# megapose6d/megapose6d

Hardware: AMD Instinct MI355X
Metric: pose-hypotheses/sec (render+coarse+refine), 640×480, megapose-1.0-RGB (higher is better)
Workload: dtype f32 (results of fp32 arithmetic; the convolutions' multiplications run on the bf16 MFMA as EXACT piece products of the fp32 operands, fp32 accumulate)

## Files before the change

### include/mp_engine_debug.h

```cpp
#ifndef MP_ENGINE_DEBUG_H
#define MP_ENGINE_DEBUG_H

#include "mp_engine.h"

#ifdef __cplusplus
extern "C" {
#endif

int mp_clock_probe(double ms_target, double* shader_mhz, double* mfma_tflops, mp_stream stream);

int mp_conv_clock_read(double* shader_mhz, int reset);

int mp_conv_wino_stats(double* direct_flops, double* executed_flops, int reset);

int mp_conv_wino_bf16_stats(double* direct_flops, double* executed_bf16_flops, int reset);
int mp_conv_wino_bf16_clock(double* shader_mhz, double* cycles_per_step, int reset);
int mp_conv_wino_bf16_phases(double* prologue_cycles, double* epilogue_cycles);
int mp_conv_wino_bf16_telemetry(int on);

int mp_conv_stem_bg_stats(double* background_wgs, double* total_wgs, int reset);

#ifdef __cplusplus
}
#endif

#endif
```

### megapose6d_amd/_lib.py

```python
from __future__ import annotations

import ctypes as C
import os
from pathlib import Path

_HERE = Path(__file__).resolve().parent
LIB_PATH = _HERE / "libmp_engine.so"


class EngineError(RuntimeError):
    pass


class MeshDesc(C.Structure):
    _fields_ = [
        ("h_vertices", C.c_void_p),
        ("h_normals", C.c_void_p),
        ("h_colors", C.c_void_p),
        ("h_faces", C.c_void_p),
        ("n_vertices", C.c_int32),
        ("n_faces", C.c_int32),
    ]


# ... 61 lines not shown
    "mp_profile_query_ex": (_i, [_i, C.c_char_p, _i, C.POINTER(_i64), C.POINTER(C.c_double), C.POINTER(C.c_double), C.POINTER(C.c_double),
                                 C.POINTER(C.c_double), C.POINTER(C.c_double)]),
    "mp_device_info": (_i, [C.POINTER(_i), C.POINTER(_i), C.c_char_p, _i]),
    "mp_mesh_db_create": (_i, [C.POINTER(MeshDesc), _i, C.POINTER(_vp)]),
    "mp_mesh_db_set_texture": (_i, [_vp, _i, _vp, _vp, _i, _i, _i]),
    "mp_mesh_db_destroy": (_i, [_vp]),
    "mp_mesh_db_max_vertices": (_i, [_vp]),
    "mp_mesh_db_radius": (_f, [_vp, _i]),
    "mp_raster_workspace_bytes": (_sz, [_vp, _i, _i, _i]),
    "mp_raster_render": (_i, [_vp, _vp, _vp, _vp, _i, _i, _i, _u32, C.POINTER(Lights), _vp, _i64, _i, _i64, _i64, _i64, _i, _i, _i,
                              _vp, _sz, _vp]),
    "mp_raster_render_crop": (_i, [_vp, _vp, _vp, _vp, _i, _i, _i, _u32, C.POINTER(Lights), _vp, _i64, _i, _i64, _i64, _i64, _i, _i, _i,
                                   _vp, _sz, _vp, _i, _i, _i, _i, _i, _vp, _vp, _i, _vp]),
    "mp_raster_render_xrec": (_i, [_vp, _vp, _vp, _vp, _i, _i, _i, _u32, C.POINTER(Lights), _vp, _i64, _i, _i64, _i64, _i64, _i, _i, _i,
                                   _vp, _sz, _vp, _i, _i, _i, _i, _i, _vp, _vp, _u32, _vp, _i, _vp]),
    "mp_raster_job_flags": (_vp, [_vp, _vp, _i, _i, _i]),
    "mp_pack_observation_nhwc4": (_i, [_vp, _i, _i, _i, _i, _vp, _vp]),
    "mp_raster_scene_workspace_bytes": (_sz, [_vp, _i, _i, _i]),
    "mp_raster_render_scene": (_i, [_vp, _i, C.POINTER(C.c_int32), _vp, _vp, _vp, _vp, _vp, _vp, _i, _i, _u32, _vp, _i64, _i64, _i64, _i, _i,
                                    _i, _vp, _vp, _sz, _vp]),
    "mp_crop_roi_align": (_i, [_vp, _i, _i, _i, _i, _vp, _vp, _i, _i, _i, _vp, _i64, _i64, _i64, _i, _vp]),
    "mp_normalize_depth": (_i, [_vp, _i, _i, _i, _i, _i, C.POINTER(C.c_int32), _i, _vp, _i, _vp]),
    "mp_normalize_depth_f16": (_i, [_vp, _i, _i, _i, _i, _i, C.POINTER(C.c_int32), _i, _vp, _i, _vp]),
    "mp_conv_packed_floats": (_sz, [_i, _i, _i, _i]),
    "mp_conv_pack_weights": (_i, [_vp, _i, _i, _i, _i, _i, _vp, _vp]),
    "mp_conv2d_nhwc": (_i, [C.POINTER(ConvDesc), _vp]),
    "mp_conv2d_plan": (_i, [C.POINTER(ConvDesc), _i, C.POINTER(C.c_int32)]),
    "mp_conv_bf16x9_packed_bytes": (_sz, [_i, _i, _i, _i]),
    "mp_conv_bf16x9_pack_weights": (_i, [_vp, _i, _i, _i, _i, _i, _vp, _vp]),
    "mp_conv2d_bf16x9_nhwc": (_i, [C.POINTER(ConvDesc), _vp, _vp]),
    "mp_conv2d_kernel_name": (C.c_char_p, [C.POINTER(ConvDesc)]),
    "mp_conv_wino_packed_floats": (_sz, [_i, _i]),
    "mp_conv_wino_pack_weights": (_i, [_vp, _i, _i, _i, _vp, _vp]),
    "mp_conv_wino_eligible": (_i, [C.POINTER(ConvDesc), _i]),
    "mp_conv3x3_wino_nhwc": (_i, [C.POINTER(ConvDesc), _vp, _vp]),
    "mp_conv_wino_stats": (_i, [C.POINTER(C.c_double), C.POINTER(C.c_double), _i]),
    "mp_conv_wino_bf16_packed_bytes": (_sz, [_i, _i]),
    "mp_conv_wino_bf16_pack_weights": (_i, [_vp, _i, _i, _i, _vp, _vp]),
    "mp_conv3x3_wino_bf16_nhwc": (_i, [C.POINTER(ConvDesc), _vp, _vp]),
    "mp_conv_wino_bf16_stats": (_i, [C.POINTER(C.c_double), C.POINTER(C.c_double), _i]),
    "mp_conv_wino_bf16_clock": (_i, [C.POINTER(C.c_double), C.POINTER(C.c_double), _i]),
    "mp_conv_wino_bf16_phases": (_i, [C.POINTER(C.c_double), C.POINTER(C.c_double)]),
    "mp_conv_wino_bf16_telemetry": (_i, [_i]),
    "mp_xrec_elements": (_i, [_i, _i]),
    "mp_conv_stem_supported": (_i, [_i, _i, _i]),
    "mp_conv_stem_packed_bytes": (_sz, [_i, _i, _i, _i]),
    "mp_conv_stem_pack_weights": (_i, [_vp, _i, _i, _i, _i, _vp, _vp]),
    "mp_conv_stem_pack_weights_mask": (_i, [_vp, _i, _i, _i, _u32, _vp, _vp]),
    "mp_conv_stem_sparse_chunks": (_i, [_i, _i, _i]),
    "mp_conv_stem_sparse_packed_bytes": (_sz, [_i, _i, _i, _i]),
    "mp_conv_stem_pack_weights_sparse": (_i, [_vp, _i, _i, _i, _i, _vp, _vp]),
    "mp_conv_stem_xrec_sparse": (_i, [C.POINTER(ConvDesc), _vp, _vp, _i, _vp, _vp, _i, _vp]),
    "mp_conv_stem_bg_stats": (_i, [C.POINTER(C.c_double), C.POINTER(C.c_double), _i]),
    "mp_conv_stem_xrec": (_i, [C.POINTER(ConvDesc), _vp, _i, _vp]),
    "mp_conv_stem_xrec_pool": (_i, [C.POINTER(ConvDesc), _vp, _i, _vp, _i, _vp]),
    "mp_maxpool3x3s2": (_i, [_vp, _i, _i, _i, _i, _i, _vp, _i, _vp, _vp, _vp, _vp]),
    "mp_bn_relu_nhwc": (_i, [_vp, _i, _i, _i, _i, _i, _vp, _vp, _vp, _vp]),
    "mp_pool_fc_heads": (_i, [_vp, _i, _i, _i, _i, _i, _vp, _vp, _i, _vp, _vp, _i, _vp, _vp, _vp, _vp]),
    "mp_backbone_create": (_i, [_i, _i, _i, _i, C.POINTER(NamedTensor), _i, C.POINTER(_vp)]),
    "mp_backbone_create_wide": (_i, [_i, _i, _i, _i, _i, C.POINTER(NamedTensor), _i, C.POINTER(_vp)]),
    "mp_backbone_destroy": (_i, [_vp]),
    "mp_backbone_input_channels_padded": (_i, [_vp]),
    "mp_backbone_input_border": (_i, [_vp]),
    "mp_backbone_workspace_bytes": (_sz, [_vp, _i, _i, _i]),
    "mp_backbone_workspace_reset": (_i, [_vp, _vp]),
    "mp_backbone_forward": (_i, [_vp, _vp, _i, _i, _i, _vp, _vp, _vp, _vp, _sz, _vp]),
    "mp_backbone_forward_f16": (_i, [_vp, _vp, _i, _i, _i, _vp, _vp, _vp, _vp, _sz, _vp]),
    "mp_backbone_xrec_elements": (_i, [_vp, _i]),
    "mp_backbone_forward_xrec": (_i, [_vp, _vp, _i, _i, _i, _i, _vp, _vp, _vp, _vp, _sz, _vp]),
    "mp_backbone_xrec_prepare": (_i, [_vp, _u32]),
    "mp_backbone_forward_xrec_mask": (_i, [_vp, _vp, _u32, _i, _i, _i, _vp, _vp, _vp, _vp, _sz, _vp]),
    "mp_backbone_forward_xrec_sparse": (_i, [_vp, _vp, _u32, _vp, _i, _i, _i, _vp, _vp, _vp, _vp, _sz, _vp]),
    "mp_backbone_flops": (C.c_double, [_vp, _i, _i, _i]),
    "mp_normalize_T": (_i, [_vp, _i, _vp, _vp]),
    "mp_init_extents": (_i, [_vp, _i, _i, _vp, _i, _vp, _vp]),
    "mp_init_poses_from_boxes": (_i, [_vp, _vp, _vp, _vp, _vp, _i, _vp, _i, _vp, _vp]),
    "mp_pose_prepare": (_i, [_vp, _vp, _vp, _vp, _i, _i, _i, _i, _i, _i, _i, _i, _i, _i, _f, _vp, _vp, _vp, _vp, _vp, _vp,
                             _vp]),
    "mp_pose_multiview_n_views": (_i, [_i]),
    "mp_pose_prepare_ex": (_i, [_vp, _vp, _vp, _vp, _i, _i, _i, _i, _i, _i, _i, _i, _i, _i, _f, _vp, _vp, _vp, _vp, _vp, _vp, _vp, _vp]),
    "mp_pose_error_workspace_bytes": (_sz, [_i, _i, _i]),
    "mp_pose_error_sym": (_i, [_vp, _vp, _vp, _vp, _i, _vp, _i, _vp, _vp, _i, _i, _i, _i, _vp, _vp, _vp, _vp, _vp, _vp, _vp, _sz, _vp]),
    "mp_pose_error_nn": (_i, [_vp, _vp, _vp, _i, _vp, _vp, _i, _i, _i, _vp, _vp, _vp, _vp, _vp, _sz, _vp]),
    "mp_pose_error_rigid": (_i, [_vp, _vp, _i, _vp, _vp, _i, _vp, _vp, _i, _vp, _vp, _vp, _vp]),
    "mp_pose_error_mspd": (_i, [_vp, _vp, _vp, _vp, _i, _vp, _i, _vp, _vp, _i, _i, _i, _i, _vp, _vp, _vp, _vp, _vp, _vp, _vp, _sz, _vp]),
    "mp_vsd_workspace_bytes": (_sz, [_i, _i]),
    "mp_vsd": (_i, [_vp, _vp, _vp, _vp, _vp, _vp, _i, _i, _i, _vp, _vp, _i, _i, _i, _f, _vp, _i, _i, _i, _vp, _vp, _vp, _sz, _vp]),
    "mp_gt_info_workspace_bytes": (_sz, [_i]),
    "mp_gt_info": (_i, [_vp, _vp, _vp, _vp, _i, _i, _vp, _i, _i, _i, _i, _f, _i, _vp, _vp, _vp, _vp, _vp, _vp, _sz, _vp]),
    "mp_bop_match_limits": (_i, [C.POINTER(_i), C.POINTER(_i), C.POINTER(_i), C.POINTER(_i)]),
    "mp_bop_match_workspace_bytes": (_sz, [_i, _i, _i]),
    "mp_bop_match": (_i, [_vp, _vp, _vp, _vp, _vp, _vp, _vp, _vp, _vp, _vp, _i, _i, _i, _i, _i, _i, _i, _vp, _vp, _sz, _vp]),
    "mp_icp_workspace_bytes": (_sz, [_i, _i, _i, _i]),
    "mp_icp_refine": (_i, [_vp, _i, _vp, _vp, _vp, _vp, _vp, _i, _i, _i, _i, _i, _f, _i, _i, _vp, _vp, _vp, _vp, _sz, _vp]),
    "mp_icp_nn_max_points": (_i, []),
    "mp_icp_nn_workspace_bytes": (_sz, [_i, _i, _i, _i]),
    "mp_icp_refine_nn": (_i, [_vp, _i, _vp, _vp, _vp, _vp, _vp, _i, _i, _i, _i, _i, _f, _i, _vp, _vp, _vp, _vp, _vp, _vp, _sz, _vp]),
    "mp_pose_update": (_i, [_vp, _vp, _i, _vp, _vp, _i, _vp, _vp]),
    "mp_detector_default_config": (_i, [C.POINTER(DetectorConfig), _i, _i, _i]),
    "mp_detector_state_spec": (_i, [_i, _i, C.c_char_p, _i, C.POINTER(_i64), C.POINTER(C.c_int32)]),
    "mp_detector_create": (_i, [C.POINTER(DetectorConfig), C.POINTER(NamedTensor), _i, C.POINTER(_vp)]),
    "mp_detector_destroy": (_i, [_vp]),
    "mp_detector_workspace_bytes": (_sz, [_vp, _i, _i, _i]),
    "mp_detector_forward": (_i, [_vp, _vp, _i, _i, _i, _vp, _vp, _vp, _vp, _vp, _vp, _sz, _vp]),
    "mp_detector_debug_tensor": (_i, [_vp, C.c_char_p, C.POINTER(_vp), C.POINTER(_i64), C.POINTER(C.c_int32), C.POINTER(_i64), C.POINTER(_i64)]),
}
# ... 34 lines not shown
```

### megapose6d_amd/csrc/conv_stem.hip

```cpp
#include <cstdlib>
#include <vector>

#include "bf16x9_split.h"
#include "common.h"

namespace mp {
namespace stem {

typedef float f32x4 __attribute__((ext_vector_type(4)));
typedef __bf16 bf16x8 __attribute__((ext_vector_type(8)));
typedef unsigned u32x4 __attribute__((ext_vector_type(4)));

constexpr int TH = 8, TW = 16;
constexpr int NCO = 64;

struct Params {
  const unsigned char* __restrict__ x;
  const unsigned char* __restrict__ w;
  const float* __restrict__ bias;
  float* __restrict__ y;
  int N, Ho, Wo;
  int Hp, Wp;
  int in_off;
  int Cout, Hop, Wop, out_border;
  int tiles_x, tiles_y, n_cb;
  int n_steps;
  int relu;
  unsigned img_bytes;
  unsigned out_bytes;
  float* __restrict__ ypool;
  int Hq, Wq, pool_border;
  const unsigned char* __restrict__ tile_flags;
  const unsigned char* __restrict__ w_sparse;
  int fl_tx, fl_ty, q_use, n_steps_sparse;
  int H, W, pad;
  int count_bg;
};

__device__ unsigned long long g_stem_bg[2];

constexpr size_t LDS_PER_WG = 80 * 1024;

template <int KS, int Q>
struct Geo {
  static constexpr int PH = 2 * (TH - 1) + KS, PW = 2 * (TW - 1) + KS;
  static constexpr int QP = (Q % 2 == 0 && (size_t)(PH + 1) * ((PW * (Q + 1)) | 1) * 16 <= LDS_PER_WG) ? Q + 1 : Q;
  static constexpr int ROW16 = PW * QP;
  static constexpr int PITCH16 = ROW16 | 1;
  static constexpr int PITCH = PITCH16 * 16;
  static constexpr int KWQ = KS * Q;
  static constexpr int S = KS * KWQ;
  static constexpr int T = ((S + 3) / 4 + 1) / 2 * 2;
  static constexpr size_t PATCH = (size_t)(PH + 1) * PITCH;
  static constexpr size_t OUT_TILE = (size_t)TH * TW * NCO * 4;
  static constexpr size_t LDS = PATCH > OUT_TILE ? PATCH : OUT_TILE;
  static_assert(4 * T + 4 - S <= KWQ, "padding slices (and the look-ahead read past the last step) must stay inside the extra row");
  static_assert(LDS <= LDS_PER_WG, "the patch must leave room for a second workgroup on the CU");
};

template <int KS, int Q, bool POOL, bool SP = false>
__global__ __launch_bounds__(256) __attribute__((amdgpu_waves_per_eu(2, 2))) void conv_stem_bf16x3(Params p) {
  using G = Geo<KS, Q>;
  extern __shared__ __attribute__((aligned(16))) unsigned char lds[];
  const int tid = threadIdx.x, lane = tid & 63;
  const int wave = __builtin_amdgcn_readfirstlane(tid >> 6);
  int wg = xcd_remap(blockIdx.x, gridDim.x);
  const int cb = wg % p.n_cb; wg /= p.n_cb;
  const int tx = wg % p.tiles_x; wg /= p.tiles_x;
  const int ty = wg % p.tiles_y;
  const int n = wg / p.tiles_y;
  bool sparse = false;
  if constexpr (SP) {
    const int r0 = max(2 * ty * TH - p.pad, 0) >> 3, r1 = min(2 * ty * TH - p.pad + G::PH - 1, p.H - 1) >> 3;
    const int c0 = max(2 * tx * TW - p.pad, 0) >> 3, c1 = min(2 * tx * TW - p.pad + G::PW - 1, p.W - 1) >> 3;
    const int nc = c1 - c0 + 1, cnt = (r1 - r0 + 1) * nc;
    unsigned char f = 0;
    if (lane < cnt) f = p.tile_flags[((size_t)n * p.fl_ty + r0 + lane / nc) * p.fl_tx + c0 + lane % nc];
    sparse = cnt <= 64 && __ballot(f != 0) == 0ull;
  }
  if constexpr (SP) {
    if (p.count_bg && tid == 0) {
      if (sparse) atomicAdd(&g_stem_bg[0], 1ull);
      if (blockIdx.x == 0) atomicAdd(&g_stem_bg[1], (unsigned long long)gridDim.x);
    }
  }
  const int QU = SP && sparse ? p.q_use : Q;
  const int n_steps = SP && sparse ? p.n_steps_sparse : p.n_steps;

  {
    const unsigned char* img = p.x + (size_t)n * p.img_bytes;
    const __amdgpu_buffer_rsrc_t r_x = __builtin_amdgcn_make_buffer_rsrc((void*)img, 0, p.img_bytes, 0x00020000);
    const int row_bytes = p.Wp * (16 * Q);
    const int org = (2 * ty * TH + p.in_off) * row_bytes + (2 * tx * TW + p.in_off) * (16 * Q);
    constexpr int SRC16 = G::PW * Q;
    constexpr int N_CH = G::PH * SRC16, PER = (N_CH + 255) / 256;
    constexpr int HALF = (PER + 1) / 2;
    u32x4 v[HALF];
#pragma unroll
    for (int h = 0; h < 2; ++h) {
#pragma unroll
      for (int k = 0; k < HALF; ++k) {
        const int c = tid + 256 * (h * HALF + k);
        const int row = c / SRC16, col = c - row * SRC16;
        const bool want = c < N_CH && (!SP || col % Q < QU);
        v[k] = want ? __builtin_amdgcn_raw_buffer_load_b128(r_x, org + row * row_bytes + col * 16, 0, 0) : u32x4{0, 0, 0, 0};
      }
#pragma unroll
      for (int k = 0; k < HALF; ++k) {
        const int c = tid + 256 * (h * HALF + k);
        const int row = c / SRC16, col = c - row * SRC16;
        const int lcol = G::QP == Q ? col : col + (col / Q) * (G::QP - Q);
        if (c < N_CH && (!SP || col % Q < QU)) *reinterpret_cast<u32x4*>(lds + row * G::PITCH + lcol * 16) = v[k];
      }
    }
    for (int c = tid; c < G::PITCH16; c += 256) *reinterpret_cast<u32x4*>(lds + G::PH * G::PITCH + c * 16) = u32x4{0, 0, 0, 0};
  }

  const size_t w_wave = ((size_t)cb * 4 + wave) * n_steps * 3072;
  const __amdgpu_buffer_rsrc_t r_w = __builtin_amdgcn_make_buffer_rsrc((void*)((SP && sparse ? p.w_sparse : p.w) + w_wave), 0, (unsigned)n_steps * 3072u, 0x00020000);
  const int w_voff = lane * 16;
  u32x4 b0[3], b1[3];
#pragma unroll
  for (int q = 0; q < 3; ++q) {
    b0[q] = __builtin_amdgcn_raw_buffer_load_b128(r_w, w_voff, q * 1024, 0);
    b1[q] = __builtin_amdgcn_raw_buffer_load_b128(r_w, w_voff, 3072 + q * 1024, 0);
  }

  const int i = lane & 15, g = lane >> 4;
  int s_r = g;
  int a_row = (2 * i) * (16 * G::QP);
  const int kwq = SP ? KS * QU : G::KWQ;
  const int qu_m = 1024 / QU + 1;
  auto slice_off = [&](int sr) {
    if constexpr (SP) {
      const int kw = (sr * qu_m) >> 10;
      return (kw * G::QP + (sr - kw * QU)) * 16;
    } else {
      return G::QP == Q ? sr * 16 : (sr + (sr / Q) * (G::QP - Q)) * 16;
    }
  };
  int a_off = a_row + slice_off(s_r);
  auto advance = [&]() {
    s_r += 4;
    if (s_r >= kwq) { s_r -= kwq; a_row += G::PITCH; }
    a_off = a_row + slice_off(s_r);
  };
  f32x4 acc[TH];
#pragma unroll
  for (int j = 0; j < TH; ++j) acc[j] = f32x4{0.f, 0.f, 0.f, 0.f};
  u32x4 a0[TH], a1[TH];

  __syncthreads();
#pragma unroll
  for (int j = 0; j < TH; ++j) a0[j] = *reinterpret_cast<const u32x4*>(lds + a_off + j * 2 * G::PITCH);
  advance();

  const int n_pairs = n_steps >> 1;
  for (int tp = 0; tp < n_pairs; ++tp) {
    const int w_next = (2 * tp + 2) * 3072;
#pragma unroll
    for (int j = 0; j < TH; ++j) a1[j] = *reinterpret_cast<const u32x4*>(lds + a_off + j * 2 * G::PITCH);
    advance();
#pragma unroll
    for (int q = 0; q < 3; ++q) {
      const bf16x8 bq = __builtin_bit_cast(bf16x8, b0[q]);
#pragma unroll
      for (int j = 0; j < TH; ++j) acc[j] = __builtin_amdgcn_mfma_f32_16x16x32_bf16(__builtin_bit_cast(bf16x8, a0[j]), bq, acc[j], 0, 0, 0);
    }
#pragma unroll
    for (int q = 0; q < 3; ++q) b0[q] = __builtin_amdgcn_raw_buffer_load_b128(r_w, w_voff, w_next + q * 1024, 0);
#pragma unroll
    for (int j = 0; j < TH; ++j) a0[j] = *reinterpret_cast<const u32x4*>(lds + a_off + j * 2 * G::PITCH);
    advance();
#pragma unroll
    for (int q = 0; q < 3; ++q) {
      const bf16x8 bq = __builtin_bit_cast(bf16x8, b1[q]);
#pragma unroll
      for (int j = 0; j < TH; ++j) acc[j] = __builtin_amdgcn_mfma_f32_16x16x32_bf16(__builtin_bit_cast(bf16x8, a1[j]), bq, acc[j], 0, 0, 0);
    }
#pragma unroll
    for (int q = 0; q < 3; ++q) b1[q] = __builtin_amdgcn_raw_buffer_load_b128(r_w, w_voff, w_next + 3072 + q * 1024, 0);
  }

  __syncthreads();
  {
    const int co = cb * NCO + wave * 16 + i;
    const float bias = p.bias ? p.bias[co] : 0.f;
    float* tile = reinterpret_cast<float*>(lds);
#pragma unroll
    for (int j = 0; j < TH; ++j)
#pragma unroll
      for (int r = 0; r < 4; ++r) {
        float v = acc[j][r] + bias;
        if (p.relu) v = fmaxf(v, 0.f);
        tile[(j * TW + 4 * g + r) * NCO + wave * 16 + i] = v;
      }
  }
  __syncthreads();
  if constexpr (POOL) {
    const int oy0 = ty * TH, ox0 = tx * TW;
    const int Hqp = p.Hq + 2 * p.pool_border, Wqp = p.Wq + 2 * p.pool_border;
    const float4* tile4 = reinterpret_cast<const float4*>(lds);
    for (int item = tid; item < (TH / 2 + 1) * (TW / 2 + 1) * 16; item += 256) {
      const int part = item & 15, pp = item >> 4;
      const int ppy = pp / (TW / 2 + 1), ppx = pp - ppy * (TW / 2 + 1);
      const int PY = ty * (TH / 2) + ppy, PX = tx * (TW / 2) + ppx;
      if (PY >= p.Hq || PX >= p.Wq) continue;
      const int wr0 = max(2 * PY - 1, 0), wr1 = min(2 * PY + 1, p.Ho - 1), wc0 = max(2 * PX - 1, 0), wc1 = min(2 * PX + 1, p.Wo - 1);
      const int r0 = max(wr0, oy0), r1 = min(wr1, oy0 + TH - 1), c0 = max(wc0, ox0), c1 = min(wc1, ox0 + TW - 1);
      if (r0 > r1 || c0 > c1) continue;
      float4 m = make_float4(0.f, 0.f, 0.f, 0.f);
      for (int r = r0; r <= r1; ++r)
        for (int c = c0; c <= c1; ++c) {
          const float4 v = tile4[((r - oy0) * TW + (c - ox0)) * 16 + part];
          m.x = fmaxf(m.x, v.x); m.y = fmaxf(m.y, v.y); m.z = fmaxf(m.z, v.z); m.w = fmaxf(m.w, v.w);
        }
      float* dst = p.ypool + ((((size_t)n * Hqp + PY + p.pool_border) * Wqp + PX + p.pool_border) * p.Cout + cb * NCO + part * 4);
      if (r0 == wr0 && r1 == wr1 && c0 == wc0 && c1 == wc1) {
        *reinterpret_cast<float4*>(dst) = m;
      } else {
        unsigned* du = reinterpret_cast<unsigned*>(dst);
        atomicMax(du, __float_as_uint(m.x) & 0x7FFFFFFFu); atomicMax(du + 1, __float_as_uint(m.y) & 0x7FFFFFFFu);
        atomicMax(du + 2, __float_as_uint(m.z) & 0x7FFFFFFFu); atomicMax(du + 3, __float_as_uint(m.w) & 0x7FFFFFFFu);
      }
    }
  }
  if (!POOL || p.y != nullptr) {
    const __amdgpu_buffer_rsrc_t r_y = __builtin_amdgcn_make_buffer_rsrc((void*)(p.y + (size_t)n * (p.out_bytes / 4)), 0, p.out_bytes, 0x00020000);
    const int oy0 = ty * TH, ox0 = tx * TW;
#pragma unroll
    for (int k = 0; k < (TH * TW * NCO / 4) / 256; ++k) {
      const int c = tid + 256 * k;
      const int pix = c >> 4, part = c & 15;
      const int oy = oy0 + (pix >> 4), ox = ox0 + (pix & 15);
      const u32x4 v = *reinterpret_cast<const u32x4*>(lds + c * 16);
      const int off = ((oy + p.out_border) * p.Wop + ox + p.out_border) * p.Cout + cb * NCO + part * 4;
      const unsigned voff = (oy < p.Ho && ox < p.Wo) ? (unsigned)off * 4u : 0xFFFFFFF0u;
      __builtin_amdgcn_raw_buffer_store_b128(v, r_y, (int)voff, 0, 0);
    }
  }
}

__host__ __device__ inline int pool_zero_positions(int Hq, int Wq) {
  const int rows4 = (Hq + TH / 2 - 1) / (TH / 2), cols8 = (Wq + TW / 2 - 1) / (TW / 2);
  return rows4 * Wq + (Hq - rows4) * cols8;
}
__global__ __launch_bounds__(256) void pool_zero_kernel(float* __restrict__ y, int N, int Hq, int Wq, int C, int border) {
  const int c4n = C / 4;
  const int P = pool_zero_positions(Hq, Wq);
  const long idx = (long)blockIdx.x * blockDim.x + threadIdx.x;
  if (idx >= (long)N * P * c4n) return;
  const int c4 = (int)(idx % c4n);
  long t = idx / c4n;
  const int pos = (int)(t % P), n = (int)(t / P);
  const int rows4 = (Hq + TH / 2 - 1) / (TH / 2), cols8 = (Wq + TW / 2 - 1) / (TW / 2);
  int py, px;
  if (pos < rows4 * Wq) {
    py = (pos / Wq) * (TH / 2);
    px = pos % Wq;
  } else {
    const int q = pos - rows4 * Wq, k = q / cols8;
    py = k + k / (TH / 2 - 1) + 1;
    px = (q % cols8) * (TW / 2);
  }
  *reinterpret_cast<float4*>(y + ((((size_t)n * (Hq + 2 * border) + py + border) * (Wq + 2 * border) + px + border) * C + c4 * 4)) =
      make_float4(0.f, 0.f, 0.f, 0.f);
}

template <int KS, int Q, bool POOL = false, bool SP = false>
int launch(const Params& p, hipStream_t s, double flops, double bytes, const char* name) {
  const double executed = 2.0 * (double)p.N * p.tiles_y * p.tiles_x * (TH * TW) * p.Cout * (double)p.n_steps * 32.0 * 3.0;
  using G = Geo<KS, Q>;
  static int attr_dev = -1;
  int dev = 0;
  MP_CHECK_HIP(hipGetDevice(&dev));
  if (attr_dev != dev) {
    MP_CHECK_HIP(hipFuncSetAttribute((const void*)conv_stem_bf16x3<KS, Q, POOL, SP>, hipFuncAttributeMaxDynamicSharedMemorySize, (int)G::LDS));
    attr_dev = dev;
  }
  if (POOL) {
    ProfScope prof0("pool_zero", 0.0, 16.0 * p.N * (p.Hq / 4 + 1) * p.Wq * p.Cout, s);
    const long total = (long)p.N * pool_zero_positions(p.Hq, p.Wq) * (p.Cout / 4);
    hipLaunchKernelGGL(pool_zero_kernel, dim3((unsigned)((total + 255) / 256)), dim3(256), 0, s, p.ypool, p.N, p.Hq, p.Wq, p.Cout, p.pool_border);
  }
  ProfScope prof(name, flops, bytes, s, executed, 2500.0);
  hipLaunchKernelGGL((conv_stem_bf16x3<KS, Q, POOL, SP>), dim3((unsigned)((long)p.N * p.tiles_y * p.tiles_x * p.n_cb)), dim3(256), G::LDS, s, p);
  MP_CHECK_HIP(hipGetLastError());
  return MP_OK;
}

inline int n_steps(int KS, int Q) { return ((KS * KS * Q + 3) / 4 + 1) / 2 * 2; }

}
}

using namespace mp;

extern "C" int mp_xrec_elements(int n_f32, int n_u8) {
  if (n_f32 < 0 || n_u8 < 0 || n_f32 + n_u8 <= 0) return 0;
  return (3 * n_f32 + n_u8 + 7) / 8 * 8;
}

extern "C" int mp_conv_stem_supported(int KS, int n_f32, int n_u8) {
  const int R = mp_xrec_elements(n_f32, n_u8);
  return (KS == 7 || KS == 5) && R >= 16 && R <= 48 ? 1 : 0;
}

extern "C" size_t mp_conv_stem_packed_bytes(int KS, int n_f32, int n_u8, int Cout) {
  const int Q = mp_xrec_elements(n_f32, n_u8) / 8;
  return (size_t)(Cout / stem::NCO) * 4 * stem::n_steps(KS, Q) * 3072;
}

extern "C" int mp_conv_stem_pack_weights(const float* w, int Cout, int Cin, int KS, int n_f32, const float* scale, void* packed) {
  MP_REQUIRE(n_f32 >= 0 && n_f32 <= 32 && n_f32 <= Cin, "mp_conv_stem_pack_weights: bad n_f32");
  return mp_conv_stem_pack_weights_mask(w, Cout, Cin, KS, n_f32 >= 32 ? 0xFFFFFFFFu : (1u << n_f32) - 1u, scale, packed);
}

static int pack_weights_walk(const float* w, int Cout, int Cin, int KS, uint32_t f32_mask, const float* scale, void* packed, int q_walk);

extern "C" int mp_conv_stem_pack_weights_mask(const float* w, int Cout, int Cin, int KS, uint32_t f32_mask, const float* scale, void* packed) {
  return pack_weights_walk(w, Cout, Cin, KS, f32_mask, scale, packed, 0);
}

extern "C" int mp_conv_stem_sparse_chunks(int KS, int n_f32, int n_u8) {
  if (!mp_conv_stem_supported(KS, n_f32, n_u8) || n_f32 <= 0) return 0;
  const int Q = mp_xrec_elements(n_f32, n_u8) / 8, q_use = (3 * n_f32 + 7) / 8;
  if (q_use >= Q) return 0;
  const int pad = 4 * stem::n_steps(KS, q_use) + 4 - KS * KS * q_use;
  return pad <= KS * q_use ? q_use : 0;
}
extern "C" size_t mp_conv_stem_sparse_packed_bytes(int KS, int n_f32, int n_u8, int Cout) {
  const int q_use = mp_conv_stem_sparse_chunks(KS, n_f32, n_u8);
  return q_use ? (size_t)(Cout / stem::NCO) * 4 * stem::n_steps(KS, q_use) * 3072 : 0;
}
extern "C" int mp_conv_stem_pack_weights_sparse(const float* w, int Cout, int Cin, int KS, int n_f32, const float* scale, void* packed) {
  const int q_use = mp_conv_stem_sparse_chunks(KS, n_f32, Cin - n_f32);
  MP_REQUIRE(q_use > 0, "mp_conv_stem_pack_weights_sparse: this record has no background-tile form");
  return pack_weights_walk(w, Cout, Cin, KS, n_f32 >= 32 ? 0xFFFFFFFFu : (1u << n_f32) - 1u, scale, packed, q_use);
}

static int pack_weights_walk(const float* w, int Cout, int Cin, int KS, uint32_t f32_mask, const float* scale, void* packed, int q_walk) {
  MP_REQUIRE(Cin >= 1 && Cin <= 32 && (Cin == 32 || (f32_mask >> Cin) == 0u), "mp_conv_stem_pack_weights_mask: mask names channels >= Cin (<= 32 input channels)");
  const int n_f32 = __builtin_popcount(f32_mask), n_u8 = Cin - n_f32;
  MP_REQUIRE(w && packed && n_u8 >= 0 && Cout % stem::NCO == 0 && mp_conv_stem_supported(KS, n_f32, n_u8),
             "mp_conv_stem_pack_weights: bad arguments (Cout %% 64, KS 5 | 7, 16 <= record <= 48 elements)");
  int ch_of_f32[32], ch_of_u8[32];
  for (int c = 0, a = 0, b = 0; c < Cin; ++c) {
    if ((f32_mask >> c) & 1u) ch_of_f32[a++] = c; else ch_of_u8[b++] = c;
  }
// ... 3 lines not shown
  memset(out, 0, (size_t)(Cout / stem::NCO) * 4 * T * 3072);
  for (int co = 0; co < Cout; ++co) {
    const int cb = co / stem::NCO, wave = (co % stem::NCO) / 16, i = co % 16;
    const double sc = scale ? (double)scale[co] : 1.0;
    for (int s = 0; s < S; ++s) {
      const int t = s / 4, g = s % 4;
      const int kh = s / (KS * Q), rr = s % (KS * Q), kw = rr / Q, q = rr % Q;
      for (int e = 0; e < 8; ++e) {
        const int slot = 8 * q + e;
        int ch;
        double f;
        if (slot < 3 * n_f32) { ch = ch_of_f32[slot / 3]; f = sc; }
        else if (slot < 3 * n_f32 + n_u8) { ch = ch_of_u8[slot - 3 * n_f32]; f = sc / 255.0; }
        else continue;
        const float v = (float)((double)w[(((size_t)co * Cin + ch) * KS + kh) * KS + kw] * f);
        unsigned short pc[3];
        bf16x9_split3(v, pc);
        for (int piece = 0; piece < 3; ++piece)
          out[((((size_t)(cb * 4 + wave) * T + t) * 3 + piece) * 64 + (g * 16 + i)) * 8 + e] = pc[piece];
      }
    }
  }
  return MP_OK;
}

static int stem_xrec_impl(const mp_conv_desc* d, const void* d_packed, int n_f32, float* d_ypool, int pool_border, mp_stream stream,
                          const void* d_packed_sparse = nullptr, const unsigned char* d_tile_flags = nullptr) {
  MP_REQUIRE(d && d->d_x && d_packed && (d->d_y || d_ypool), "mp_conv_stem_xrec: null pointer");
  MP_REQUIRE(!d_ypool || (d->relu && pool_border >= 0), "mp_conv_stem_xrec_pool: the fused max pool needs the ReLU (its atomicMax orders non-negative floats)");
  const int n_u8 = d->c_real - n_f32;
  MP_REQUIRE(d->KH == d->KW && d->stride == 2 && d->Cout % stem::NCO == 0 && !d->d_residual && !d->d_y_act && d->in_border >= d->pad &&
                 mp_conv_stem_supported(d->KH, n_f32, n_u8),
             "mp_conv_stem_xrec: unsupported layer (square 5x5 / 7x7, stride 2, Cout %% 64, c_real = real channels, 16 <= record <= 48 elements)");
  const int R = mp_xrec_elements(n_f32, n_u8), Q = R / 8;
  stem::Params p;
  p.x = (const unsigned char*)d->d_x; p.w = (const unsigned char*)d_packed; p.bias = d->d_bias; p.y = d->d_y;
  p.N = d->N;
  p.Ho = (d->H + 2 * d->pad - d->KH) / 2 + 1; p.Wo = (d->W + 2 * d->pad - d->KW) / 2 + 1;
  p.Hp = d->H + 2 * d->in_border; p.Wp = d->W + 2 * d->in_border; p.in_off = d->in_border - d->pad;
  p.Cout = d->Cout; p.Hop = p.Ho + 2 * d->out_border; p.Wop = p.Wo + 2 * d->out_border; p.out_border = d->out_border;
  p.tiles_x = ceil_div(p.Wo, stem::TW); p.tiles_y = ceil_div(p.Ho, stem::TH); p.n_cb = d->Cout / stem::NCO;
  p.n_steps = stem::n_steps(d->KH, Q);
  p.relu = d->relu;
  const long img = (long)p.Hp * p.Wp * 16 * Q, outb = (long)p.Hop * p.Wop * d->Cout * 4;
  MP_REQUIRE(img < (1L << 31) && outb < (1L << 31) && (long)d->N * p.tiles_y * p.tiles_x * p.n_cb < (1L << 31), "mp_conv_stem_xrec: image too large for 32-bit offsets");
  p.img_bytes = (unsigned)img; p.out_bytes = (unsigned)outb;
  p.ypool = d_ypool; p.pool_border = pool_border;
  p.Hq = (p.Ho + 2 - 3) / 2 + 1; p.Wq = (p.Wo + 2 - 3) / 2 + 1;
  p.H = d->H; p.W = d->W; p.pad = d->pad;
  p.tile_flags = nullptr; p.w_sparse = nullptr; p.fl_tx = p.fl_ty = 0; p.q_use = Q; p.n_steps_sparse = p.n_steps;
  const int q_use = mp_conv_stem_sparse_chunks(d->KH, n_f32, n_u8);
  const bool sp = d_packed_sparse && d_tile_flags && q_use > 0;
  p.count_bg = 0;
  if (sp) {
    p.count_bg = mp_profile_active();
    p.tile_flags = d_tile_flags; p.w_sparse = (const unsigned char*)d_packed_sparse;
    p.fl_tx = ceil_div(d->W, 8); p.fl_ty = ceil_div(d->H, 8); p.q_use = q_use; p.n_steps_sparse = stem::n_steps(d->KH, q_use);
  }
  const double M = (double)d->N * p.Ho * p.Wo;
  const double flops = 2.0 * M * d->Cout * d->KH * d->KW * d->c_real;
  const double bytes = (double)d->N * img + (d->d_y ? 4.0 * M * d->Cout : 0.0) + (d_ypool ? 4.0 * (double)d->N * p.Hq * p.Wq * d->Cout : 0.0) +
                       (double)mp_conv_stem_packed_bytes(d->KH, n_f32, n_u8, d->Cout);
  hipStream_t s = (hipStream_t)stream;
#define MP_STEM_GO(KSV, QV)                                                                                                          \
  if (d->KH == KSV && Q == QV) {                                                                                                   \
    if (sp)                                                                                                                        \
      return d_ypool ? stem::launch<KSV, QV, true, true>(p, s, flops, bytes, "conv_stem_bf16x3+maxpool<" #KSV "x" #KSV ",Q" #QV ">")   \
                     : stem::launch<KSV, QV, false, true>(p, s, flops, bytes, "conv_stem_bf16x3<" #KSV "x" #KSV ",Q" #QV ">");       \
    return d_ypool ? stem::launch<KSV, QV, true>(p, s, flops, bytes, "conv_stem_bf16x3+maxpool<" #KSV "x" #KSV ",Q" #QV ">")         \
                   : stem::launch<KSV, QV, false>(p, s, flops, bytes, "conv_stem_bf16x3<" #KSV "x" #KSV ",Q" #QV ">");               \
  }
  MP_STEM_GO(7, 2) MP_STEM_GO(7, 3) MP_STEM_GO(7, 4) MP_STEM_GO(7, 5) MP_STEM_GO(7, 6)
  MP_STEM_GO(5, 2) MP_STEM_GO(5, 3) MP_STEM_GO(5, 4) MP_STEM_GO(5, 5) MP_STEM_GO(5, 6)
#undef MP_STEM_GO
  set_error("mp_conv_stem_xrec: no instance for %dx%d, record of %d elements", d->KH, d->KW, R);
  return MP_ERR_INVALID;
}

extern "C" int mp_conv_stem_xrec(const mp_conv_desc* d, const void* d_packed, int n_f32, mp_stream stream) {
  MP_REQUIRE(d && d->d_y, "mp_conv_stem_xrec: null output");
  return stem_xrec_impl(d, d_packed, n_f32, nullptr, 0, stream);
}

extern "C" int mp_conv_stem_xrec_pool(const mp_conv_desc* d, const void* d_packed, int n_f32, float* d_ypool, int pool_border, mp_stream stream) {
  MP_REQUIRE(d_ypool, "mp_conv_stem_xrec_pool: null pooled output");
  return stem_xrec_impl(d, d_packed, n_f32, d_ypool, pool_border, stream);
}

extern "C" int mp_conv_stem_xrec_sparse(const mp_conv_desc* d, const void* d_packed, const void* d_packed_sparse, int n_f32,
                                        const unsigned char* d_tile_flags, float* d_ypool, int pool_border, mp_stream stream) {
  MP_REQUIRE(d && (d->d_y || d_ypool), "mp_conv_stem_xrec_sparse: null output");
  return stem_xrec_impl(d, d_packed, n_f32, d_ypool, pool_border, stream, d_packed_sparse, d_tile_flags);
}

extern "C" int mp_conv_stem_bg_stats(double* background_wgs, double* total_wgs, int reset) {
  unsigned long long h[2] = {0, 0};
  MP_CHECK_HIP(hipDeviceSynchronize());
  MP_CHECK_HIP(hipMemcpyFromSymbol(h, HIP_SYMBOL(stem::g_stem_bg), sizeof(h)));
  if (background_wgs) *background_wgs = (double)h[0];
  if (total_wgs) *total_wgs = (double)h[1];
  if (reset) {
    const unsigned long long z[2] = {0, 0};
    MP_CHECK_HIP(hipMemcpyToSymbol(HIP_SYMBOL(stem::g_stem_bg), z, sizeof(z)));
  }
  return MP_OK;
}
```

### megapose6d_amd/engine.py

```python
from __future__ import annotations

import ctypes as C
from typing import Dict, List, Optional, Sequence, Tuple

import numpy as np
import torch

from . import _lib
from ._lib import ConvDesc, EngineError, Lights, MeshDesc, NamedTensor, check

RASTER_NORMALS = 1
RASTER_DEPTH = 2
RASTER_NORMALS_GL = 4
RASTER_MSAA4 = 16
RASTER_F16 = 32
RASTER_XREC = 64

BACKBONE_KINDS = {"vanilla_resnet34": 0, "resnet34": 1, "resnet18": 2}


def _stream() -> int:
    return torch.cuda.current_stream().cuda_stream


# ... 363 lines not shown

def conv_wino_bf16_stats(reset: bool = True) -> Tuple[float, float]:
    a, b = C.c_double(0), C.c_double(0)
    check(_lib.load().mp_conv_wino_bf16_stats(C.byref(a), C.byref(b), 1 if reset else 0))
    return a.value, b.value


def conv_wino_bf16_clock(reset: bool = True) -> Tuple[float, float]:
    a, b = C.c_double(0), C.c_double(0)
    check(_lib.load().mp_conv_wino_bf16_clock(C.byref(a), C.byref(b), 1 if reset else 0))
    return a.value, b.value


def leading_mask(n_f32: int) -> int:
    return (1 << int(n_f32)) - 1


def conv_stem_pack_weights(w_oihw: np.ndarray, n_f32: int, scale: Optional[np.ndarray] = None, f32_mask: Optional[int] = None) -> np.ndarray:
    lib = _lib.load()
    w = np.ascontiguousarray(w_oihw, dtype=np.float32)
    Cout, Cin, KH, KW = w.shape
    assert KH == KW
    mask = leading_mask(n_f32) if f32_mask is None else int(f32_mask)
    nf = bin(mask).count("1")
    out = np.empty(lib.mp_conv_stem_packed_bytes(KH, nf, Cin - nf, Cout), dtype=np.uint8)
    sc = None if scale is None else np.ascontiguousarray(scale, dtype=np.float32)
    check(lib.mp_conv_stem_pack_weights_mask(w.ctypes.data, Cout, Cin, KH, mask, None if sc is None else sc.ctypes.data, out.ctypes.data))
    return out


def xrec_elements(n_f32: int, n_u8: int) -> int:
    return int(_lib.load().mp_xrec_elements(n_f32, n_u8))


def conv_stem_pack_weights_sparse(w_oihw: np.ndarray, n_f32: int, scale: Optional[np.ndarray] = None) -> Optional[np.ndarray]:
    lib = _lib.load()
    w = np.ascontiguousarray(w_oihw, dtype=np.float32)
    Cout, Cin, KH, KW = w.shape
    n = lib.mp_conv_stem_sparse_packed_bytes(KH, n_f32, Cin - n_f32, Cout)
    if n == 0:
        return None
    out = np.empty(n, dtype=np.uint8)
    sc = None if scale is None else np.ascontiguousarray(scale, dtype=np.float32)
    check(lib.mp_conv_stem_pack_weights_sparse(w.ctypes.data, Cout, Cin, KH, n_f32, None if sc is None else sc.ctypes.data, out.ctypes.data))
    return out


def conv_stem_bg_stats(reset: bool = True) -> Tuple[float, float]:
    a, b = C.c_double(), C.c_double()
    check(_lib.load().mp_conv_stem_bg_stats(C.byref(a), C.byref(b), int(reset)))
    return a.value, b.value


def conv_stem_xrec(xrec: torch.Tensor, N: int, H: int, W: int, c_real: int, n_f32: int, in_border: int, w_pieces: torch.Tensor,
                   bias: Optional[torch.Tensor], Cout: int, K: int, pad: int, y: Optional[torch.Tensor], out_border: int, relu: bool = False,
                   y_pool: Optional[torch.Tensor] = None, pool_border: int = 1, w_sparse: Optional[torch.Tensor] = None,
                   tile_flags: Optional[torch.Tensor] = None) -> None:
    assert xrec.dtype == torch.bfloat16 and w_pieces.dtype == torch.uint8
    d = ConvDesc()
    d.d_x, d.N, d.H, d.W, d.C, d.c_real, d.in_border = xrec.data_ptr(), N, H, W, (c_real + 3) // 4 * 4, c_real, in_border
    d.d_bias = _ptr(bias)
    d.Cout, d.KH, d.KW, d.stride, d.pad = Cout, K, K, 2, pad
    d.d_y, d.out_border, d.relu = _ptr(y), out_border, int(relu)
    if w_sparse is not None and tile_flags is not None:
        assert tile_flags.dtype == torch.uint8 and tile_flags.is_cuda and w_sparse.dtype == torch.uint8
        check(_lib.load().mp_conv_stem_xrec_sparse(C.byref(d), w_pieces.data_ptr(), w_sparse.data_ptr(), n_f32, tile_flags.data_ptr(),
                                                   _ptr(y_pool), pool_border, _stream()))
        return
    if y_pool is not None:
        check(_lib.load().mp_conv_stem_xrec_pool(C.byref(d), w_pieces.data_ptr(), n_f32, y_pool.data_ptr(), pool_border, _stream()))
        return
    check(_lib.load().mp_conv_stem_xrec(C.byref(d), w_pieces.data_ptr(), n_f32, _stream()))


def conv2d_plan(N: int, H: int, W: int, Cp: int, in_border: int, Cout: int, K: int, stride: int, pad: int, n_cu: int,
                ws_floats: int = 0, x_f16: bool = False) -> Dict[str, int]:
    d = ConvDesc()
    d.x_f16 = int(x_f16)
    dummy = 0x1000
    d.d_x, d.N, d.H, d.W, d.C, d.in_border = dummy, N, H, W, Cp, in_border
    d.d_w, d.Cout, d.KH, d.KW, d.stride, d.pad = dummy, Cout, K, K, stride, pad
    d.d_y, d.out_border = dummy, 1
    if ws_floats:
        d.d_splitk_ws, d.splitk_ws_floats = dummy, ws_floats
    out = (C.c_int32 * 5)()
    check(_lib.load().mp_conv2d_plan(C.byref(d), n_cu, out))
    return dict(zip(("mode", "k_split", "chunks_per_split", "n_main", "m_begin"), out))


def maxpool3x3s2(x, N, H, W, Cc, in_border, y, out_border, y_act=None, sc=None, sh=None) -> None:
    check(_lib.load().mp_maxpool3x3s2(x.data_ptr(), N, H, W, Cc, in_border, _ptr(y), out_border, _ptr(y_act), _ptr(sc), _ptr(sh),
                                      _stream()))


def bn_relu_nhwc(x, N, H, W, Cc, border, y_act, sc, sh) -> None:
    check(_lib.load().mp_bn_relu_nhwc(x.data_ptr(), N, H, W, Cc, border, y_act.data_ptr(), sc.data_ptr(), sh.data_ptr(), _stream()))


def pool_fc_heads(x, N, H, W, Cc, in_border, fc_w, fc_b, n_feat, head_w, head_b, n_out, feat, out, sigmoid) -> None:
    check(_lib.load().mp_pool_fc_heads(x.data_ptr(), N, H, W, Cc, in_border, _ptr(fc_w), _ptr(fc_b), n_feat, head_w.data_ptr(),
                                       head_b.data_ptr(), n_out, _ptr(feat), out.data_ptr(), _ptr(sigmoid), _stream()))


class Backbone:

    def __init__(self, kind: str, c_in: int, head: str, n_out: int, state_dict: Dict[str, torch.Tensor]):
# ... 498 lines not shown
```

Measured before the change: 2340.

## Overlap stem patch loads with weight prefetch and split fused pool into interior/rim

The stem convolution now issues every input-patch buffer load at once and then starts the weight prefetch before writing the patch into LDS. Loads for unwanted chunks are sent to an out-of-range offset rather than masked. The fused max-pool splits into an interior pass, which writes float4 results directly without atomics, and a per-lane rim pass that uses atomicMax only on pool windows that cross a tile edge and skips zero values. The change also adds optional cycle-counter telemetry per phase, at the cost of more registers for the staged loads and two extra branches on the telemetry flag.

```diff
diff --git a/include/mp_engine_debug.h b/include/mp_engine_debug.h
--- a/include/mp_engine_debug.h
+++ b/include/mp_engine_debug.h
@@ -19,6 +19,8 @@
 int mp_conv_wino_bf16_telemetry(int on);
 
 int mp_conv_stem_bg_stats(double* background_wgs, double* total_wgs, int reset);
+int mp_conv_stem_telemetry(int on);
+int mp_conv_stem_phases(int KS, int Q, double* dense, double* background, int reset);
 
 #ifdef __cplusplus
 }
diff --git a/megapose6d_amd/_lib.py b/megapose6d_amd/_lib.py
--- a/megapose6d_amd/_lib.py
+++ b/megapose6d_amd/_lib.py
@@ -137,6 +137,8 @@
     "mp_conv_stem_pack_weights_sparse": (_i, [_vp, _i, _i, _i, _i, _vp, _vp]),
     "mp_conv_stem_xrec_sparse": (_i, [C.POINTER(ConvDesc), _vp, _vp, _i, _vp, _vp, _i, _vp]),
     "mp_conv_stem_bg_stats": (_i, [C.POINTER(C.c_double), C.POINTER(C.c_double), _i]),
+    "mp_conv_stem_telemetry": (_i, [_i]),
+    "mp_conv_stem_phases": (_i, [_i, _i, C.POINTER(C.c_double), C.POINTER(C.c_double), _i]),
     "mp_conv_stem_xrec": (_i, [C.POINTER(ConvDesc), _vp, _i, _vp]),
     "mp_conv_stem_xrec_pool": (_i, [C.POINTER(ConvDesc), _vp, _i, _vp, _i, _vp]),
     "mp_maxpool3x3s2": (_i, [_vp, _i, _i, _i, _i, _i, _vp, _i, _vp, _vp, _vp, _vp]),
diff --git a/megapose6d_amd/csrc/conv_stem.hip b/megapose6d_amd/csrc/conv_stem.hip
--- a/megapose6d_amd/csrc/conv_stem.hip
+++ b/megapose6d_amd/csrc/conv_stem.hip
@@ -1,3 +1,4 @@
+#include <atomic>
 #include <cstdlib>
 #include <vector>
 
@@ -35,9 +36,15 @@
   int fl_tx, fl_ty, q_use, n_steps_sparse;
   int H, W, pad;
   int count_bg;
+  int telemetry;
+  int tel_slot;
 };
 
 __device__ unsigned long long g_stem_bg[2];
+
+constexpr int STEM_N_STAMPS = 6, STEM_N_INST = 10;
+__device__ unsigned long long g_stem_phase[STEM_N_INST][2][8];
+#define STEM_STAMP(K) if (tel) tc[K] = __builtin_readcyclecounter();
 
 constexpr size_t LDS_PER_WG = 80 * 1024;
 
@@ -64,6 +71,9 @@
   extern __shared__ __attribute__((aligned(16))) unsigned char lds[];
   const int tid = threadIdx.x, lane = tid & 63;
   const int wave = __builtin_amdgcn_readfirstlane(tid >> 6);
+  const bool tel = p.telemetry != 0 && (blockIdx.x & 63) == 0 && wave == 0;
+  unsigned long long tc0 = 0, tc[STEM_N_STAMPS] = {};
+  if (tel) tc0 = __builtin_readcyclecounter();
   int wg = xcd_remap(blockIdx.x, gridDim.x);
   const int cb = wg % p.n_cb; wg /= p.n_cb;
   const int tx = wg % p.tiles_x; wg /= p.tiles_x;
@@ -87,34 +97,21 @@
   const int QU = SP && sparse ? p.q_use : Q;
   const int n_steps = SP && sparse ? p.n_steps_sparse : p.n_steps;
 
-  {
-    const unsigned char* img = p.x + (size_t)n * p.img_bytes;
-    const __amdgpu_buffer_rsrc_t r_x = __builtin_amdgcn_make_buffer_rsrc((void*)img, 0, p.img_bytes, 0x00020000);
-    const int row_bytes = p.Wp * (16 * Q);
-    const int org = (2 * ty * TH + p.in_off) * row_bytes + (2 * tx * TW + p.in_off) * (16 * Q);
-    constexpr int SRC16 = G::PW * Q;
-    constexpr int N_CH = G::PH * SRC16, PER = (N_CH + 255) / 256;
-    constexpr int HALF = (PER + 1) / 2;
-    u32x4 v[HALF];
-#pragma unroll
-    for (int h = 0; h < 2; ++h) {
-#pragma unroll
-      for (int k = 0; k < HALF; ++k) {
-        const int c = tid + 256 * (h * HALF + k);
-        const int row = c / SRC16, col = c - row * SRC16;
-        const bool want = c < N_CH && (!SP || col % Q < QU);
-        v[k] = want ? __builtin_amdgcn_raw_buffer_load_b128(r_x, org + row * row_bytes + col * 16, 0, 0) : u32x4{0, 0, 0, 0};
-      }
-#pragma unroll
-      for (int k = 0; k < HALF; ++k) {
-        const int c = tid + 256 * (h * HALF + k);
-        const int row = c / SRC16, col = c - row * SRC16;
-        const int lcol = G::QP == Q ? col : col + (col / Q) * (G::QP - Q);
-        if (c < N_CH && (!SP || col % Q < QU)) *reinterpret_cast<u32x4*>(lds + row * G::PITCH + lcol * 16) = v[k];
-      }
-    }
-    for (int c = tid; c < G::PITCH16; c += 256) *reinterpret_cast<u32x4*>(lds + G::PH * G::PITCH + c * 16) = u32x4{0, 0, 0, 0};
-  }
+  const unsigned char* img = p.x + (size_t)n * p.img_bytes;
+  const __amdgpu_buffer_rsrc_t r_x = __builtin_amdgcn_make_buffer_rsrc((void*)img, 0, p.img_bytes, 0x00020000);
+  const int row_bytes = p.Wp * (16 * Q);
+  const int org = (2 * ty * TH + p.in_off) * row_bytes + (2 * tx * TW + p.in_off) * (16 * Q);
+  constexpr int SRC16 = G::PW * Q;
+  constexpr int N_CH = G::PH * SRC16, PER = (N_CH + 255) / 256;
+  u32x4 v[PER];
+#pragma unroll
+  for (int k = 0; k < PER; ++k) {
+    const int c = tid + 256 * k;
+    const int row = c / SRC16, col = c - row * SRC16;
+    const bool want = c < N_CH && (!SP || col % Q < QU);
+    v[k] = __builtin_amdgcn_raw_buffer_load_b128(r_x, want ? org + row * row_bytes + col * 16 : (int)0xFFFFFFF0u, 0, 0);
+  }
+  STEM_STAMP(0)
 
   const size_t w_wave = ((size_t)cb * 4 + wave) * n_steps * 3072;
   const __amdgpu_buffer_rsrc_t r_w = __builtin_amdgcn_make_buffer_rsrc((void*)((SP && sparse ? p.w_sparse : p.w) + w_wave), 0, (unsigned)n_steps * 3072u, 0x00020000);
@@ -124,6 +121,14 @@
   for (int q = 0; q < 3; ++q) {
     b0[q] = __builtin_amdgcn_raw_buffer_load_b128(r_w, w_voff, q * 1024, 0);
     b1[q] = __builtin_amdgcn_raw_buffer_load_b128(r_w, w_voff, 3072 + q * 1024, 0);
+  }
+  for (int c = tid; c < G::PITCH16; c += 256) *reinterpret_cast<u32x4*>(lds + G::PH * G::PITCH + c * 16) = u32x4{0, 0, 0, 0};
+#pragma unroll
+  for (int k = 0; k < PER; ++k) {
+    const int c = tid + 256 * k;
+    const int row = c / SRC16, col = c - row * SRC16;
+    const int lcol = G::QP == Q ? col : col + (col / Q) * (G::QP - Q);
+    if (256 * (k + 1) <= N_CH || c < N_CH) *reinterpret_cast<u32x4*>(lds + row * G::PITCH + lcol * 16) = v[k];
   }
 
   const int i = lane & 15, g = lane >> 4;
@@ -151,6 +156,7 @@
   u32x4 a0[TH], a1[TH];
 
   __syncthreads();
+  STEM_STAMP(1)
 #pragma unroll
   for (int j = 0; j < TH; ++j) a0[j] = *reinterpret_cast<const u32x4*>(lds + a_off + j * 2 * G::PITCH);
   advance();
@@ -183,6 +189,7 @@
   }
 
   __syncthreads();
+  STEM_STAMP(2)
   {
     const int co = cb * NCO + wave * 16 + i;
     const float bias = p.bias ? p.bias[co] : 0.f;
@@ -197,31 +204,46 @@
       }
   }
   __syncthreads();
+  STEM_STAMP(3)
   if constexpr (POOL) {
     const int oy0 = ty * TH, ox0 = tx * TW;
     const int Hqp = p.Hq + 2 * p.pool_border, Wqp = p.Wq + 2 * p.pool_border;
+    float* const qimg = p.ypool + (size_t)n * Hqp * Wqp * p.Cout + cb * NCO;
     const float4* tile4 = reinterpret_cast<const float4*>(lds);
-    for (int item = tid; item < (TH / 2 + 1) * (TW / 2 + 1) * 16; item += 256) {
+    for (int item = tid; item < (TH / 2 - 1) * (TW / 2 - 1) * 16; item += 256) {
       const int part = item & 15, pp = item >> 4;
-      const int ppy = pp / (TW / 2 + 1), ppx = pp - ppy * (TW / 2 + 1);
+      const int ppy = 1 + pp / (TW / 2 - 1), ppx = 1 + pp % (TW / 2 - 1);
       const int PY = ty * (TH / 2) + ppy, PX = tx * (TW / 2) + ppx;
       if (PY >= p.Hq || PX >= p.Wq) continue;
-      const int wr0 = max(2 * PY - 1, 0), wr1 = min(2 * PY + 1, p.Ho - 1), wc0 = max(2 * PX - 1, 0), wc1 = min(2 * PX + 1, p.Wo - 1);
-      const int r0 = max(wr0, oy0), r1 = min(wr1, oy0 + TH - 1), c0 = max(wc0, ox0), c1 = min(wc1, ox0 + TW - 1);
-      if (r0 > r1 || c0 > c1) continue;
+      const int r0 = 2 * PY - 1, r1 = min(2 * PY + 1, p.Ho - 1), c0 = 2 * PX - 1, c1 = min(2 * PX + 1, p.Wo - 1);
       float4 m = make_float4(0.f, 0.f, 0.f, 0.f);
       for (int r = r0; r <= r1; ++r)
         for (int c = c0; c <= c1; ++c) {
           const float4 v = tile4[((r - oy0) * TW + (c - ox0)) * 16 + part];
           m.x = fmaxf(m.x, v.x); m.y = fmaxf(m.y, v.y); m.z = fmaxf(m.z, v.z); m.w = fmaxf(m.w, v.w);
         }
-      float* dst = p.ypool + ((((size_t)n * Hqp + PY + p.pool_border) * Wqp + PX + p.pool_border) * p.Cout + cb * NCO + part * 4);
+      *reinterpret_cast<float4*>(qimg + ((size_t)(PY + p.pool_border) * Wqp + PX + p.pool_border) * p.Cout + part * 4) = m;
+    }
+    const float* tile = reinterpret_cast<const float*>(lds);
+    constexpr int RIM = 2 * (TW / 2 + 1) + 2 * (TH / 2 - 1);
+    for (int e = wave; e < RIM; e += 4) {
+      int ppy, ppx;
+      if (e < 2 * (TW / 2 + 1)) { ppy = e < TW / 2 + 1 ? 0 : TH / 2; ppx = e < TW / 2 + 1 ? e : e - (TW / 2 + 1); }
+      else { ppy = 1 + ((e - 2 * (TW / 2 + 1)) >> 1); ppx = ((e - 2 * (TW / 2 + 1)) & 1) * (TW / 2); }
+      const int PY = ty * (TH / 2) + ppy, PX = tx * (TW / 2) + ppx;
+      if (PY >= p.Hq || PX >= p.Wq) continue;
+      const int wr0 = max(2 * PY - 1, 0), wr1 = min(2 * PY + 1, p.Ho - 1), wc0 = max(2 * PX - 1, 0), wc1 = min(2 * PX + 1, p.Wo - 1);
+      const int r0 = max(wr0, oy0), r1 = min(wr1, oy0 + TH - 1), c0 = max(wc0, ox0), c1 = min(wc1, ox0 + TW - 1);
+      if (r0 > r1 || c0 > c1) continue;
+      float m = 0.f;
+      for (int r = r0; r <= r1; ++r)
+        for (int c = c0; c <= c1; ++c) m = fmaxf(m, tile[((r - oy0) * TW + (c - ox0)) * NCO + lane]);
+      float* dst = qimg + ((size_t)(PY + p.pool_border) * Wqp + PX + p.pool_border) * p.Cout + lane;
       if (r0 == wr0 && r1 == wr1 && c0 == wc0 && c1 == wc1) {
-        *reinterpret_cast<float4*>(dst) = m;
+        *dst = m;
       } else {
-        unsigned* du = reinterpret_cast<unsigned*>(dst);
-        atomicMax(du, __float_as_uint(m.x) & 0x7FFFFFFFu); atomicMax(du + 1, __float_as_uint(m.y) & 0x7FFFFFFFu);
-        atomicMax(du + 2, __float_as_uint(m.z) & 0x7FFFFFFFu); atomicMax(du + 3, __float_as_uint(m.w) & 0x7FFFFFFFu);
+        const unsigned u = __float_as_uint(m) & 0x7FFFFFFFu;
+        if (u != 0u) atomicMax(reinterpret_cast<unsigned*>(dst), u);
       }
     }
   }
@@ -237,6 +259,19 @@
       const int off = ((oy + p.out_border) * p.Wop + ox + p.out_border) * p.Cout + cb * NCO + part * 4;
       const unsigned voff = (oy < p.Ho && ox < p.Wo) ? (unsigned)off * 4u : 0xFFFFFFF0u;
       __builtin_amdgcn_raw_buffer_store_b128(v, r_y, (int)voff, 0, 0);
+    }
+  }
+  if (tel) {
+    tc[4] = __builtin_readcyclecounter();
+    __builtin_amdgcn_s_waitcnt(0);
+    tc[5] = __builtin_readcyclecounter();
+    if (lane == 0) {
+      unsigned long long* g = g_stem_phase[p.tel_slot][SP && sparse ? 1 : 0];
+      unsigned long long prev = tc0;
+#pragma unroll
+      for (int k = 0; k < STEM_N_STAMPS; ++k) { atomicAdd(&g[k], tc[k] - prev); prev = tc[k]; }
+      atomicAdd(&g[6], tc[5] - tc0);
+      atomicAdd(&g[7], 1ull);
     }
   }
 }
@@ -295,6 +330,8 @@
 }
 
 using namespace mp;
+
+static std::atomic<int> g_stem_telemetry{0};
 
 extern "C" int mp_xrec_elements(int n_f32, int n_u8) {
   if (n_f32 < 0 || n_u8 < 0 || n_f32 + n_u8 <= 0) return 0;
@@ -404,6 +441,8 @@
   const int q_use = mp_conv_stem_sparse_chunks(d->KH, n_f32, n_u8);
   const bool sp = d_packed_sparse && d_tile_flags && q_use > 0;
   p.count_bg = 0;
+  p.telemetry = g_stem_telemetry.load(std::memory_order_relaxed);
+  p.tel_slot = (d->KH == 5 ? 5 : 0) + Q - 2;
   if (sp) {
     p.count_bg = mp_profile_active();
     p.tile_flags = d_tile_flags; p.w_sparse = (const unsigned char*)d_packed_sparse;
@@ -457,3 +496,22 @@
   }
   return MP_OK;
 }
+
+extern "C" int mp_conv_stem_telemetry(int on) { return g_stem_telemetry.exchange(on ? 1 : 0); }
+
+extern "C" int mp_conv_stem_phases(int KS, int Q, double* dense, double* background, int reset) {
+  MP_REQUIRE((KS == 7 || KS == 5) && Q >= 2 && Q <= 6, "mp_conv_stem_phases: no such instance (KS 5 | 7, Q 2 .. 6)");
+  static unsigned long long h[stem::STEM_N_INST][2][8];
+  MP_CHECK_HIP(hipDeviceSynchronize());
+  MP_CHECK_HIP(hipMemcpyFromSymbol(h, HIP_SYMBOL(stem::g_stem_phase), sizeof(h)));
+  const int slot = (KS == 5 ? 5 : 0) + Q - 2;
+  for (int k = 0; k < 8; ++k) {
+    if (dense) dense[k] = (double)h[slot][0][k];
+    if (background) background[k] = (double)h[slot][1][k];
+  }
+  if (reset) {
+    memset(h[slot], 0, sizeof(h[slot]));
+    MP_CHECK_HIP(hipMemcpyToSymbol(HIP_SYMBOL(stem::g_stem_phase), h, sizeof(h)));
+  }
+  return MP_OK;
+}
diff --git a/megapose6d_amd/engine.py b/megapose6d_amd/engine.py
--- a/megapose6d_amd/engine.py
+++ b/megapose6d_amd/engine.py
@@ -439,6 +439,19 @@
     return a.value, b.value
 
 
+STEM_PHASES = ("requests", "resident", "k_loop", "tile", "issue", "retire")
+
+
+def conv_stem_telemetry(on: bool) -> bool:
+    return bool(_lib.load().mp_conv_stem_telemetry(int(bool(on))))
+
+
+def conv_stem_phases(K: int, Q: int, reset: bool = True) -> Dict[str, Dict[str, float]]:
+    a, b = (C.c_double * 8)(), (C.c_double * 8)()
+    check(_lib.load().mp_conv_stem_phases(K, Q, a, b, int(reset)))
+    return {kind: {**dict(zip(STEM_PHASES, v[:6])), "total": v[6], "workgroups": v[7]} for kind, v in (("dense", list(a)), ("background", list(b)))}
+
+
 def conv_stem_xrec(xrec: torch.Tensor, N: int, H: int, W: int, c_real: int, n_f32: int, in_border: int, w_pieces: torch.Tensor,
                    bias: Optional[torch.Tensor], Cout: int, K: int, pad: int, y: Optional[torch.Tensor], out_border: int, relu: bool = False,
                    y_pool: Optional[torch.Tensor] = None, pool_border: int = 1, w_sparse: Optional[torch.Tensor] = None,
```

After: 2327. Within noise of the previous version (-0.5%).
